# kit4b/kit4b

Measured on AMD Instinct MI355X. Metric: Mreads/sec aligned (100 bp SE vs 3 Gbp .sfx), higher is better.
Workload: dtype u64

## Files before the change

### kit4b_amd/csrc/k4_align.hip

```cpp
#include <stdlib.h>
#include <type_traits>
#include "k4_align_common.h"

#define K4_BS(nch) ((nch) >= 16 ? 128 : 256)
template <int NCH>
struct K4Lane {
  const uint64_t* rd;
  uint32_t* ded;
  const uint32_t* sup;
  const uint64_t* ent;
  uint64_t* memo;
  static constexpr int NW = NCH + 1;
  K4_DEV uint64_t word(int s, int c) const { return rd[(s * NW + c) * K4_BS(NCH)]; }
  K4_DEV uint64_t chunk_at(int s, int o) const {
    int w = o >> 5, sh = 2 * (o & 31);
    uint64_t hi = word(s, w);
    if (!sh) return hi;
    return (hi << sh) | (word(s, w + 1) >> (64 - sh));
  }
};

struct K4Probe {
  int cmp;
  int mm;
// ... 110 lines not shown
      more = cnt == PFN;
      bool memo_hit = false, memo_pending = false;
      int memo_mm = 0;
#pragma unroll
      for (int j = 0; j < PFN; j++) {
        if (j < cnt) {
          if (!CAPTURE && j == 0 && first_group && tshift == 0 && (sizeof(KT) == 4 || cl >= kk + 2)) {
            const uint64_t mv = ln.memo[s * K4_BS(NCH)];
            const int kind = (int)(mv >> 62), fm = (int)((mv >> 48) & 0x3FFF), mmv = (int)((mv >> 40) & 0xFF);
            if (kind == 1 || (kind == 2 && fm < cl)) continue;
            if (kind == 2 && mmv != 0xFF) {
              lb0[0] = 0; lb1[0] = 1; ps0[0] = (RT)(mv & 0xFFFFFFFFFFull);
              memo_hit = true; memo_mm = mmv;
              continue;
            }
          }
          const uint64_t code = ln.chunk_at(s, oo[j]) >> (64 - 2 * kk);
          uint64_t sub;
          {
            KT e_lb0, e_ps0, e_lb1;
            k4d_ktab_fetch<KT>(ix, code << tshift, (code + 1) << tshift, e_lb0, e_ps0, sig[j], e_lb1, sub,
                               sizeof(KT) == 8 && tshift == 0 && cl >= kk + 2);
            lb0[j] = (RT)e_lb0; ps0[j] = (RT)e_ps0; lb1[j] = (RT)e_lb1;
          }
          if (CAPTURE && defer_deep && tshift == 0 && (uint64_t)(lb1[j] - lb0[j]) > K4_DEFER_BUCKET) return K4_DEFER;
          if (a.deep_general && (!CAPTURE || a.deep_general == 1) && tshift == 0 && (uint64_t)(lb1[j] - lb0[j]) > K4_DEFER_BUCKET) return K4_NEED_SLOW;
          if (sizeof(KT) == 8 && tshift == 0 && cl >= kk + 2 && sub != K4_KTAB64_IRREGULAR) {
            uint32_t before, count;
            k4d_ktab_sub(sub, (uint32_t)(ln.chunk_at(s, oo[j] + kk) >> 60), before, count);
            if (before) ps0[j] = (RT)NOPOS;
            lb0[j] += (RT)before;
            lb1[j] = lb0[j] + (RT)count;
          }
          if (CAPTURE && j == 0 && first_group && tshift == 0) {
            if (lb1[0] == lb0[0]) ln.memo[s * K4_BS(NCH)] = k4d_memo_pack(1, 0, 0, 0);
            else memo_pending = lb1[0] == lb0[0] + 1;
          }
          if (sizeof(KT) == 4 && tshift == 0 && lb1[j] == lb0[j] + 1 && cl > kk) {
            const int nb = min(K4_SIG_BASES32, cl - kk);
            const uint32_t cb = (uint32_t)(ln.chunk_at(s, oo[j] + kk) >> 32);
            const uint32_t df = (cb ^ sig[j]) & (0xFFFFFFFFu << (32 - 2 * nb));
            if (df) {
              lb1[j] = lb0[j];
              if (CAPTURE && j == 0 && first_group) {
                ln.memo[s * K4_BS(NCH)] = k4d_memo_pack(2, (uint64_t)ps0[0], 0xFF, kk + (__clz(df) >> 1));
                memo_pending = false;
              }
            }
          }
        }
      }
      uint32_t touch = 0;
#pragma unroll
      for (int j = 0; j < PFN; j++)
        if (j < cnt && tshift == 0 && lb1[j] > lb0[j] && !(j == 0 && memo_hit) && (sizeof(KT) == 4 || (uint64_t)ps0[j] != NOPOS))
          touch |= ix.ref2[((int64_t)ps0[j] - oo[j]) >> 4];

#pragma unroll
      for (int j = 0; j < PFN; j++) {
        if (j >= cnt || stop) continue;
        const int o = oo[j];
        n_lookup++;
        int64_t lo = (int64_t)lb0[j];
        int64_t hi = (int64_t)lb1[j] - 1;
        const int64_t bucket_hi = hi;
        int64_t found = -1;
        uint64_t fpos = 0;
        int fmm = 0;
        while (lo <= hi) {
          const int64_t mid = (lo + hi) >> 1;
          const uint64_t p = (tshift == 0 && mid == (int64_t)lb0[j] && (sizeof(KT) == 4 || (uint64_t)ps0[j] != NOPOS))
                                 ? (uint64_t)ps0[j] : k4d_sa_at<EL>(ix, (uint64_t)mid);
          K4Probe pr;
          if (!CAPTURE && j == 0 && memo_hit) { pr.cmp = 0; pr.mm = memo_mm; pr.fm = len; pr.exc = false; }
          else {
            pr = k4d_probe<NCH>(ix, ln, s, o, cl, len, p);
            n_probe++;
            if (CAPTURE && j == 0 && memo_pending) ln.memo[s * K4_BS(NCH)] = k4d_memo_pack(2, p, pr.mm > 254 ? 254 : pr.mm, pr.fm);
          }
          if (pr.exc) return K4_NEED_SLOW;
          if (pr.cmp > 0) lo = mid + 1;
          else {
            if (pr.cmp == 0) { found = mid; fpos = p; fmm = pr.mm; }
            hi = mid - 1;
          }
        }
        if (found != lo) continue;
        int64_t idx = found;
        uint64_t p = fpos;
        int mm = fmm;
        int iter = 0;
        bool first = true;
        while (!max_iter || iter < max_iter) {
          if (!first) {
            if (idx >= bucket_hi || idx + 1 >= n) break;
            const uint64_t p2 = k4d_sa_at<EL>(ix, (uint64_t)idx + 1);
            if ((int64_t)p2 + cl > n) break;
            const K4Probe pr = k4d_probe<NCH>(ix, ln, s, o, cl, len, p2);
            n_probe++;
            if (pr.exc) return K4_NEED_SLOW;
            if (pr.cmp != 0) break;
            idx += 1; p = p2; mm = pr.mm;
          }
          first = false;
          if (p < (uint64_t)o) continue;
          const uint64_t left = p - (uint64_t)o;
          int e;
          uint64_t e_start, e_end;
          if (ix.n_entries <= K4_LDS_ENTRIES) {
            int lo_e = 0, hi_e = (int)ix.n_entries - 1;
            e = -1; e_start = 0; e_end = 0;
            while (hi_e >= lo_e) {
              const int mid_e = (hi_e + lo_e) >> 1;
              const uint64_t sv = ln.ent[mid_e];
              if (sv > left) { hi_e = mid_e - 1; continue; }
              const uint64_t ev = ln.ent[K4_LDS_ENTRIES + mid_e];
              if (ev >= left) { e = mid_e; e_start = sv; e_end = ev; break; }
              lo_e = mid_e + 1;
            }
          } else {
            e = k4d_map_entry(ix, left);
            e_start = e >= 0 ? ix.ent_start[e] : 0;
            e_end = e >= 0 ? ix.ent_end[e] : 0;
          }
          if (e < 0 || left + (uint64_t)len - 1 > e_end) continue;
          const uint32_t targ_id = (uint32_t)(1 + p - (uint32_t)o);
          bool dup = false;
          for (int q = 0; q < n_ded; q++) dup |= (ln.ded[q * K4_BS(NCH)] == targ_id);
          if (dup) continue;
          if (n_ded >= K4_DEDUP_CAP) return K4_NEED_SLOW;
          ln.ded[n_ded * K4_BS(NCH)] = targ_id;
          n_ded++;
          iter++;
          n_cand++;
          if (mm > allow_mm || mm >= st.nxt) continue;
          k4d_fold(st, mm, hits, rp.max_hits, ix.ent_id[e], (uint32_t)(left - e_start), len, strand_c);
          if (st.inst > rp.max_hits && st.low == 0) break;
        }
        if (st.inst > rp.max_hits && st.low == 0) stop = true;
      }
      if (touch == 0x5A5A5A5Au && len < 0) n_probe++;
      first_group = false;
    }
  }
  return k4d_lcm_result(*p_inst, *p_low, p_nxt, st, rp.mm_delta, rp.max_hits, p_inst, p_low);
}

K4_DEV uint64_t k4d_rev2(uint64_t x) {
  uint64_t y = __brevll(x);
  return ((y & 0x5555555555555555ull) << 1) | ((y >> 1) & 0x5555555555555555ull);
}

template <int NCH>
K4_DEV uint32_t k4d_pack_read(const uint8_t* __restrict__ src, int len, uint64_t* col, uint32_t& n_ns) {
  constexpr int NW = NCH + 1;
  uint32_t fl = 0;
  n_ns = 0;
  const uint32_t sh = (uint32_t)(reinterpret_cast<uintptr_t>(src) & 3);
  const uint32_t* __restrict__ src32 = reinterpret_cast<const uint32_t*>(src - sh);
  const int span = len + (int)sh;
#pragma unroll
  for (int c = 0; c < NCH; c++) {
    uint64_t acc = 0;
    if (32 * c < len) {
      uint32_t dq[9] = {0, 0, 0, 0, 0, 0, 0, 0, 0};
      if (c * 32 + 32 <= span) {
        uint32_t d8[8];
        k4d_load_words<8>(src32 + c * 8, d8);
#pragma unroll
        for (int q = 0; q < 8; q++) dq[q] = d8[q];
      } else {
#pragma unroll
        for (int q = 0; q < 8; q++)
          if (c * 32 + q * 4 < span) dq[q] = src32[c * 8 + q];
      }
      if (c * 32 + 32 < span) dq[8] = src32[c * 8 + 8];
#pragma unroll
      for (int q = 0; q < 8; q++) {
        const int base = c * 32 + q * 4;
        uint32_t d = __builtin_amdgcn_alignbyte(dq[q + 1], dq[q], sh);
        d &= 0x07070707u;
        if (base + 4 > len) d &= len > base ? (0xFFFFFFFFu >> (8 * (4 - (len - base)))) : 0u;
        const uint32_t hi4 = d & 0x04040404u;
        if (hi4) {
          const uint32_t inval = hi4 & ((d << 1) | (d << 2)) & 0x04040404u;
          if (inval) fl |= K4_RF_INVALID;
          n_ns += __popc(hi4 & ~inval);
          d &= ~(hi4 | (hi4 >> 1) | (hi4 >> 2));
        }
        acc = (acc << 8) | ((d & 3) << 6) | (((d >> 8) & 3) << 4) | (((d >> 16) & 3) << 2) | ((d >> 24) & 3);
      }
    }
    col[c * K4_BS(NCH)] = acc;
  }
  col[NCH * K4_BS(NCH)] = 0;
  if (n_ns) fl |= K4_RF_HAS_N;
#pragma unroll
  for (int c = 0; c < NCH; c++) {
    uint64_t r = 0;
    if (32 * c < len) {
      const int o = len - 32 * (c + 1);
      uint64_t f;
      if (o >= 0) {
        const int w = o >> 5, sh = 2 * (o & 31);
        const uint64_t hi = col[w * K4_BS(NCH)];
        f = sh ? (hi << sh) | (col[(w + 1) * K4_BS(NCH)] >> (64 - sh)) : hi;
      } else
        f = col[0] >> (2 * (-o));
      r = k4d_rev2(~f) & k4d_range_mask(0, len - 32 * c);
    }
    col[(NW + c) * K4_BS(NCH)] = r;
  }
  col[(NW + NCH) * K4_BS(NCH)] = 0;
  return fl;
}

template <int EL, int NCH, bool FIRST, typename KT, bool DEFER = false>
__global__ void __launch_bounds__(K4_BS(NCH), (NCH >= 16 ? K4_STEP_WAVES_LONG : NCH >= 8 ? K4_STEP_WAVES_MID : NCH == 5 ? K4_STEP_WAVES_5 : K4_STEP_WAVES)) k4k_align_step(K4AlignArgs a, int step, const uint32_t* __restrict__ in_ids,
                                                      const uint64_t* __restrict__ in_rows,
                                                      const uint32_t* __restrict__ in_count, uint32_t* __restrict__ out_ids,
                                                      uint64_t* __restrict__ out_rows, uint32_t* __restrict__ out_count) {
  extern __shared__ uint64_t lds[];
  constexpr int NW = NCH + 1;
  const int tid = threadIdx.x;
  const int lane = tid & 63;
  K4Lane<NCH> ln;
  ln.rd = lds + tid;
  ln.ded = reinterpret_cast<uint32_t*>(lds + 2 * NW * K4_BS(NCH)) + tid;
  ln.memo = lds + 2 * NW * K4_BS(NCH) + (K4_DEDUP_CAP * K4_BS(NCH)) / 2 + tid;
  uint64_t* ent_l = lds + 2 * NW * K4_BS(NCH) + (K4_DEDUP_CAP * K4_BS(NCH)) / 2 + 2 * K4_BS(NCH);
  uint32_t* sup_l = reinterpret_cast<uint32_t*>(ent_l + 2 * K4_LDS_ENTRIES);
  ln.ent = ent_l;
  ln.sup = sup_l;
  for (int q = tid; q < K4_SUP_WORDS; q += K4_BS(NCH)) sup_l[q] = a.ix.excsup[q];
  if (a.ix.n_entries <= K4_LDS_ENTRIES)
    for (int q = tid; q < (int)a.ix.n_entries; q += K4_BS(NCH)) {
      ent_l[q] = a.ix.ent_start[q];
      ent_l[K4_LDS_ENTRIES + q] = a.ix.ent_end[q];
    }
  __syncthreads();
  uint64_t* col = lds + tid;
  uint32_t n_lookup = 0, n_probe = 0, n_cand = 0, n_slow = 0, n_bases = 0, n_done = 0;
  const int64_t count = (FIRST && !(DEFER && in_ids != nullptr)) ? a.n_reads : (int64_t)*in_count;
  const int64_t stride = (int64_t)gridDim.x * K4_BS(NCH);
  uint32_t ch_cur = 0, ch_left = 0;
  const bool from_list = !FIRST || (DEFER && in_ids != nullptr);
  const bool may_defer = DEFER && FIRST && in_ids == nullptr && a.defer_ids != nullptr;
  uint32_t dch_cur = 0, dch_left = 0;
  for (int64_t jb = (int64_t)blockIdx.x * K4_BS(NCH) + (tid & ~63); jb < count; jb += stride) {
    const int64_t j = jb + lane;
    bool active = j < count;
    int64_t i = 0;
    if (active) {
      i = from_list ? (int64_t)in_ids[j] : j;
      if (from_list && (uint32_t)i == K4_NO_READ) active = false;
    }
    bool slow = false, survive = false, deferred = false;
    int ext_from = -1;
    if (active) {
      const int len = (int)a.lens[i];
      const K4ReadParams rp = k4d_read_params(a, len);
      bool skip = false;
      if (FIRST) {
        if (!from_list) {
          n_done++;
          n_bases += (uint32_t)len;
        }
        uint32_t fl = 0, n_ns = 0;
        if (len < 1 || len > 32 * NCH || len > K4_MAX_FAST_READ_LEN) {
          fl = K4_RF_TOOLONG;
          if (a.mode == 1) {
            const uint8_t* src = a.reads + a.offs[i];
            for (int q = 0; q < len; q++) {
              uint32_t b = src[q] & 7;
              if (b == 4) n_ns++; else if (b > 4) fl |= K4_RF_INVALID;
            }
          }
        } else
          fl = k4d_pack_read<NCH>(a.reads + a.offs[i], len, col, n_ns);
        if (a.mode == 1) {
          int max_ns = 0;
          if (a.kp.max_ns) max_ns = max((len * a.kp.max_ns) / 100, a.kp.max_ns);
          if ((fl & K4_RF_INVALID) || (int)n_ns > max_ns) {
            k4_read_result r = {K4_HR_SEQERRS, 0, 0, 0, K4_NAR_NS, 0};
            a.rr[i] = r;
            if (!a.sparse_hits)
              for (int q = 0; q < a.max_hits; q++) *reinterpret_cast<uint4*>(&a.hits[i * a.max_hits + q]) = make_uint4(0, 0, 0, 0);
            skip = true;
          }
        }
        slow = fl != 0 && !skip;
        if (((a.mode == 1 && a.kp.pe_mode == 4) || a.best) && !skip) slow = true;
      } else {
        const uint64_t* row = in_rows + (int64_t)j * K4_ROW_WORDS(NCH);
        {
          const k4_u64x2_a8 mv = *reinterpret_cast<const k4_u64x2_a8*>(row + 2 * NCH);
          ln.memo[0] = mv.x; ln.memo[K4_BS(NCH)] = mv.y;
        }
        uint64_t rw[2 * NCH];
#pragma unroll
        for (int c = 0; c < NCH; c++) {
          const k4_u64x2_a8 v = *reinterpret_cast<const k4_u64x2_a8*>(row + 2 * c);
          rw[2 * c] = v.x; rw[2 * c + 1] = v.y;
        }
#pragma unroll
        for (int c = 0; c < NCH; c++) {
          col[c * K4_BS(NCH)] = rw[c];
          col[(NW + c) * K4_BS(NCH)] = rw[NCH + c];
        }
        col[NCH * K4_BS(NCH)] = 0;
        col[(NW + NCH) * K4_BS(NCH)] = 0;
      }
      if (!skip && (rp.core_len < 1 || rp.max_hits < 1 || rp.max_hits > a.max_hits)) slow = true;
      if (!skip && !slow) {
        int n_esc = 0;
        if (rp.tot_mm > 0)
          for (; n_esc <= rp.tot_mm; n_esc++)
            if (len / (n_esc + rp.mm_delta) <= rp.core_len) break;
        const bool has_final = rp.tot_mm > 0 ? n_esc <= rp.tot_mm : true;
        const int n_phases = n_esc + (has_final ? 1 : 0);
        int allow, cl, delta;
        if (step < n_esc) { allow = step; cl = len / (step + rp.mm_delta); delta = cl; }
        else { allow = rp.tot_mm; cl = rp.core_len; delta = rp.core_delta; }
        k4_hit* hits = a.hits + i * a.max_hits;
        int inst = 0, low = 0, nxt = 0;
        const uint32_t c0 = n_lookup, c1 = n_probe, c2 = n_cand;
        if (FIRST) { ln.memo[0] = K4_MEMO_NONE; ln.memo[K4_BS(NCH)] = K4_MEMO_NONE; }
        int rslt = k4d_lcm_fast<EL, NCH, KT, FIRST>(a, ln, len, allow, cl, delta, rp, &inst, &low, &nxt, hits, n_lookup, n_probe, n_cand, DEFER && may_defer);
        if (rslt == K4_NEED_SLOW) {
          slow = true;
          n_lookup = c0; n_probe = c1; n_cand = c2;
        }
        else if (DEFER && rslt == K4_DEFER) {
          deferred = true;
          n_lookup = c0; n_probe = c1; n_cand = c2;
        }
        else if (rslt == 0 && step + 1 >= n_phases && a.ext_on) { slow = true; ext_from = n_phases; }
        else if (rslt != 0 || step + 1 >= n_phases) k4d_finalize(a, i, len, rp, rslt, inst, low, nxt);
        else survive = true;
      }
      if (slow) {
        k4d_push_slow(a, i, ext_from >= 0 ? ext_from : step);
        n_slow++;
      }
    }
    if (FIRST && DEFER) {
      const unsigned long long dm = __ballot(deferred);
      const uint32_t dcnt = (uint32_t)__popcll(dm);
      if (dcnt) {
        if (dcnt > dch_left) {
          for (uint32_t q = lane; q < dch_left; q += 64) a.defer_ids[dch_cur + q] = K4_NO_READ;
          uint32_t base = 0;
          if (lane == 0) base = atomicAdd(&a.ctl[K4_CTL_DEFER], (uint32_t)K4_CHUNK);
          dch_cur = __shfl(base, 0, 64);
          dch_left = K4_CHUNK;
        }
        if (deferred) a.defer_ids[dch_cur + (uint32_t)__popcll(dm & ((1ull << lane) - 1ull))] = (uint32_t)i;
        dch_cur += dcnt;
        dch_left -= dcnt;
      }
    }
    const unsigned long long m = __ballot(survive);
    const uint32_t cnt = (uint32_t)__popcll(m);
    if (cnt) {
      if (cnt > ch_left) {
        for (uint32_t q = lane; q < ch_left; q += 64) out_ids[ch_cur + q] = K4_NO_READ;
        uint32_t base = 0;
        if (lane == 0) base = atomicAdd(out_count, (uint32_t)K4_CHUNK);
        ch_cur = __shfl(base, 0, 64);
        ch_left = K4_CHUNK;
      }
      if (survive) {
        const uint32_t slot = ch_cur + (uint32_t)__popcll(m & ((1ull << lane) - 1ull));
        out_ids[slot] = (uint32_t)i;
        uint64_t* row = out_rows + (int64_t)slot * K4_ROW_WORDS(NCH);
#pragma unroll
        for (int c = 0; c < NCH; c++) {
          k4_u64x2_a8 v;
          const int w0 = 2 * c, w1 = 2 * c + 1;
          v.x = w0 < NCH ? col[w0 * K4_BS(NCH)] : col[(NW + w0 - NCH) * K4_BS(NCH)];
          v.y = w1 < NCH ? col[w1 * K4_BS(NCH)] : col[(NW + w1 - NCH) * K4_BS(NCH)];
          *reinterpret_cast<k4_u64x2_a8*>(row + 2 * c) = v;
        }
        {
          k4_u64x2_a8 mv;
          mv.x = ln.memo[0]; mv.y = ln.memo[K4_BS(NCH)];
          *reinterpret_cast<k4_u64x2_a8*>(row + 2 * NCH) = mv;
        }
      }
      ch_cur += cnt;
      ch_left -= cnt;
    }
  }
  for (uint32_t q = lane; q < ch_left; q += 64) out_ids[ch_cur + q] = K4_NO_READ;
  if (FIRST && DEFER)
    for (uint32_t q = lane; q < dch_left; q += 64) a.defer_ids[dch_cur + q] = K4_NO_READ;
  {
    unsigned long long v[6] = {n_done, n_lookup, n_probe, n_cand, n_slow, n_bases};
#pragma unroll
    for (int q = 0; q < 6; q++) {
      unsigned long long x = v[q];
      for (int d = 32; d > 0; d >>= 1) x += __shfl_down(x, d, 64);
      if (lane == 0 && x) atomicAdd(&a.counters[q], x);
    }
  }
}

static uint32_t next_pow2(uint64_t v) {
  uint32_t p = 1;
  while (p < v) p <<= 1;
  return p;
}

static size_t k4_survivor_slots(size_t cap) {
  static_assert(K4_CHUNK * 7 >= 8 * 63, "cap / 7 must cover the abandoned chunk tails");
  return cap + cap / 7 + (size_t)2048 * 4 * K4_CHUNK + K4_CHUNK;
}

static int nch_for(int max_len) {
  if (max_len <= 128) return 4;
  if (max_len <= 160) return 5;
  if (max_len <= 256) return 8;
  return 16;
}

extern "C" int k4_reserve(k4_index* ix, int64_t max_reads, int32_t max_read_len, int32_t max_hits) {
  if (!ix || max_reads < 0 || max_read_len < 1 || max_hits < 1) return K4_ERR_PARAMS;
  if (max_read_len > K4_MAX_READ_LEN) return k4_fail(ix, K4_ERR_PARAMS, "read length %d exceeds %d", max_read_len, K4_MAX_READ_LEN);
  if (max_reads >= 0xFFFFFFF0ll) return k4_fail(ix, K4_ERR_PARAMS, "at most 2^32-16 reads per batch");
  K4_HIP(ix, hipSetDevice(ix->device));
  K4Workspace& w = ix->ws;
  bool touched = false;
  int fast_len = std::min<int>(max_read_len, K4_MAX_FAST_READ_LEN);
  if (max_reads > w.cap_reads || fast_len > w.cap_len) {
    int64_t cap = std::max<int64_t>(max_reads, w.cap_reads);
    cap = (cap + 255) / 256 * 256;
    int len = std::max(fast_len, w.cap_len);
    int nch = nch_for(len);
    touched = true;
    w.cap_reads = 0;
    w.cap_len = 0;
    for (void* q : {(void*)w.ids[0], (void*)w.ids[1], (void*)w.rows[0], (void*)w.rows[1], (void*)w.slow_list, (void*)w.slow_step,
                    (void*)w.huge_list, (void*)w.huge_step})
      if (q) hipFree(q);
    w.ids[0] = w.ids[1] = nullptr; w.rows[0] = w.rows[1] = nullptr; w.slow_list = nullptr; w.slow_step = nullptr;
    w.huge_list = nullptr; w.huge_step = nullptr;
    const size_t slots = k4_survivor_slots((size_t)cap);
    for (int b = 0; b < 2; b++) {
      K4_HIP(ix, hipMalloc(&w.ids[b], slots * 4));
      K4_HIP(ix, hipMalloc(&w.rows[b], slots * K4_ROW_WORDS(nch) * 8));
    }
    K4_HIP(ix, hipMalloc(&w.slow_list, (size_t)cap * 4));
    K4_HIP(ix, hipMalloc(&w.slow_step, (size_t)cap));
    K4_HIP(ix, hipMalloc(&w.huge_list, (size_t)cap * 4));
    K4_HIP(ix, hipMalloc(&w.huge_step, (size_t)cap));
    w.cap_reads = cap;
    w.cap_len = len;
  }
  if (!w.ctl) {
    touched = true;
    K4_HIP(ix, hipMalloc(&w.ctl, K4_CTL_WORDS * 4));
    K4_HIP(ix, hipMemset(w.ctl, 0, K4_CTL_WORDS * 4));
  }
  uint64_t nodes = ix->d.max_iter ? std::min<uint64_t>((uint64_t)ix->d.max_iter * 48, K4_MAX_IDENT_NODES) : K4_MAX_IDENT_NODES;
  uint32_t hcap = next_pow2(std::max<uint64_t>(2 * nodes + 2, 1024));
  if (!w.slow_hash || hcap > w.slow_hash_cap) {
    touched = true;
    if (w.slow_hash) hipFree(w.slow_hash);
    w.slow_hash = nullptr;
    const size_t words = (size_t)K4_SLOW_WAVES * K4_SMALL_HASH + (size_t)K4_HUGE_WAVES * hcap;
    const size_t bytes = words * 8 + (size_t)(K4_SLOW_WAVES + K4_HUGE_WAVES) * 4;
    K4_HIP(ix, hipMalloc(&w.slow_hash, bytes));
    K4_HIP(ix, hipMemset(w.slow_hash, 0, bytes));
    w.slow_hash_cap = hcap;
    w.slow_lanes = K4_SLOW_WAVES;
  }
  w.cap_hits = std::max(w.cap_hits, max_hits);
  if (touched) K4_HIP(ix, hipDeviceSynchronize());
  return K4_OK;
}

template <int EL, int NCH, typename KT>
static int launch_steps(k4_index* ix, K4AlignArgs& a, int n_steps, hipStream_t st) {
  K4Workspace& w = ix->ws;
  const size_t lds = (size_t)2 * (NCH + 1) * K4_BS(NCH) * 8 + (size_t)K4_DEDUP_CAP * K4_BS(NCH) * 4 + (size_t)2 * K4_BS(NCH) * 8 + (size_t)2 * K4_LDS_ENTRIES * 8 +
                     (size_t)K4_SUP_WORDS * 4 + 16;
  if (lds > 48 * 1024) {
    K4_HIP(ix, hipFuncSetAttribute((const void*)k4k_align_step<EL, NCH, true, KT, false>, hipFuncAttributeMaxDynamicSharedMemorySize, (int)lds));
    K4_HIP(ix, hipFuncSetAttribute((const void*)k4k_align_step<EL, NCH, true, KT, true>, hipFuncAttributeMaxDynamicSharedMemorySize, (int)lds));
    K4_HIP(ix, hipFuncSetAttribute((const void*)k4k_align_step<EL, NCH, false, KT>, hipFuncAttributeMaxDynamicSharedMemorySize, (int)lds));
  }
  const unsigned full = 256 * 8 * (256 / K4_BS(NCH));
  const bool timed = ix->timing && ix->ev_used < 4096;
  if (timed) {
    if (ix->ev_used == ix->ev0.size()) {
      hipEvent_t e0, e1, e2;
      K4_HIP(ix, hipEventCreate(&e0));
      K4_HIP(ix, hipEventCreate(&e1));
      K4_HIP(ix, hipEventCreate(&e2));
      ix->ev0.push_back(e0);
      ix->ev1.push_back(e1);
      ix->ev2.push_back(e2);
    }
    K4_HIP(ix, hipEventRecord(ix->ev0[ix->ev_used], st));
  }
  unsigned grid0 = (unsigned)std::min<int64_t>((a.n_reads + K4_BS(NCH) - 1) / K4_BS(NCH), full);
  static const int deep_mode = getenv("K4_DEEP_TO_GENERAL") ? atoi(getenv("K4_DEEP_TO_GENERAL")) : 0;
  a.deep_general = (deep_mode && ix->deep_bucket_frac >= K4_DEFER_MIN_FRAC) ? deep_mode : 0;
  if (ix->deep_bucket_frac >= K4_DEFER_MIN_FRAC && a.deep_general != 1) {
    a.defer_ids = w.ids[1];
    hipLaunchKernelGGL((k4k_align_step<EL, NCH, true, KT, true>), dim3(grid0), dim3(K4_BS(NCH)), lds, st, a, 0, (const uint32_t*)nullptr,
                       (const uint64_t*)nullptr, (const uint32_t*)nullptr, w.ids[0], w.rows[0], w.ctl + 2);
    hipLaunchKernelGGL((k4k_align_step<EL, NCH, true, KT, true>), dim3(grid0), dim3(K4_BS(NCH)), lds, st, a, 0, (const uint32_t*)w.ids[1],
                       (const uint64_t*)nullptr, (const uint32_t*)(w.ctl + K4_CTL_DEFER), w.ids[0], w.rows[0], w.ctl + 2);
  } else {
    a.defer_ids = nullptr;
    hipLaunchKernelGGL((k4k_align_step<EL, NCH, true, KT, false>), dim3(grid0), dim3(K4_BS(NCH)), lds, st, a, 0, (const uint32_t*)nullptr,
                       (const uint64_t*)nullptr, (const uint32_t*)nullptr, w.ids[0], w.rows[0], w.ctl + 2);
  }
  for (int t = 1; t < n_steps; t++) {
    const int in = (t - 1) & 1, out = t & 1;
    hipLaunchKernelGGL((k4k_align_step<EL, NCH, false, KT>), dim3(grid0), dim3(K4_BS(NCH)), lds, st, a, t, w.ids[in], w.rows[in],
                       w.ctl + 2 + (t - 1), w.ids[out], w.rows[out], w.ctl + 2 + t);
  }
  if (timed) K4_HIP(ix, hipEventRecord(ix->ev1[ix->ev_used], st));
  return K4_OK;
}

template <int EL, typename KT>
static int launch_all(k4_index* ix, K4AlignArgs& a, int max_len, int n_steps, hipStream_t st) {
  K4Workspace& w = ix->ws;
  const int nch = nch_for(std::min(max_len, K4_MAX_FAST_READ_LEN));
  if (nch > nch_for(w.cap_len)) return k4_fail(ix, K4_ERR_INTERNAL, "workspace not reserved for read length %d", max_len);
  if (n_steps < 1 || n_steps > K4_CTL_WORDS - 4) return k4_fail(ix, K4_ERR_INTERNAL, "bad phase count %d", n_steps);
  a.slow_list = w.slow_list;
  a.slow_step = w.slow_step;
  a.ctl = w.ctl;
  a.counters = (unsigned long long*)ix->counters;
  a.huge_list = w.huge_list;
  a.huge_step = w.huge_step;
  a.slow_probe = nullptr;
  a.slow_hash = w.slow_hash;
  a.slow_hash_cap = w.slow_hash_cap;
  a.slow_gen = reinterpret_cast<uint32_t*>(w.slow_hash + (size_t)K4_SLOW_WAVES * K4_SMALL_HASH + (size_t)K4_HUGE_WAVES * w.slow_hash_cap);
  a.nw = nch + 1;
  if (a.n_reads == 0) return K4_OK;
  K4_HIP(ix, hipMemsetAsync(w.ctl, 0, K4_CTL_WORDS * 4, st));
  int rc;
  switch (nch) {
    case 4: rc = launch_steps<EL, 4, KT>(ix, a, n_steps, st); break;
    case 5: rc = launch_steps<EL, 5, KT>(ix, a, n_steps, st); break;
    case 8: rc = launch_steps<EL, 8, KT>(ix, a, n_steps, st); break;
    default: rc = launch_steps<EL, 16, KT>(ix, a, n_steps, st); break;
  }
  if (rc != K4_OK) return rc;
  rc = k4i_launch_general(ix, a, max_len, st);
  if (rc != K4_OK) return rc;
  if (ix->timing && ix->ev_used < ix->ev0.size() && ix->ev_used < 4096) {
    K4_HIP(ix, hipEventRecord(ix->ev2[ix->ev_used], st));
    ix->ev_used++;
  }
  K4_HIP(ix, hipGetLastError());
  return K4_OK;
}

static int run_dev(k4_index* ix, K4AlignArgs& a, int max_len, void* stream) {
  K4Workspace& w = ix->ws;
  if (a.n_reads > w.cap_reads || std::min(max_len, K4_MAX_FAST_READ_LEN) > w.cap_len || a.max_hits > w.cap_hits ||
      !w.slow_hash || !w.ids[0] || !w.ids[1] || !w.rows[0] || !w.rows[1] || !w.slow_list || !w.huge_list || !w.ctl)
    return k4_fail(ix, K4_ERR_PARAMS, "k4_reserve(%lld, %d, %d) must precede the *_dev call", (long long)a.n_reads,
                   max_len, a.max_hits);
  a.ix = ix->d;
  hipStream_t st = (hipStream_t)stream;
  {
    const int mc = a.mode == 0 ? a.ap.min_chimeric_len : a.kp.min_chimeric_len;
    const int mi = a.mode == 0 ? a.ap.micro_indel_len : a.kp.micro_indel_len;
    const int ms = a.mode == 0 ? a.ap.max_splice_junct_len : a.kp.max_splice_junct_len;
    if (mc < 0 || mi < 0 || mi > 20 || ms < 0 || (ms != 0 && (ms < 25 || ms > 100000)))
      return k4_fail(ix, K4_ERR_PARAMS, "MinChimericLen / microInDelLen (0..20) / MaxSpliceJunctLen (0, 25..100000) out of range");
    a.ext_on = (mc > 0 || mi > 0 || ms > 0) ? 1 : 0;
    if ((mi > 0 || ms > 0) && !a.seg2)
      return k4_fail(ix, K4_ERR_PARAMS, "microInDel / splice phases report two segments: use the *_ext entry points (k4_seg2 output)");
    if (a.ext_on && (a.best || (a.mode == 1 && a.kp.pe_mode == 4)))
      return k4_fail(ix, K4_ERR_PARAMS, "the optional AlignReads phases cannot be combined with LocateBestMatches (-N)");
    if (a.seg2 && a.n_reads > 0) K4_HIP(ix, hipMemsetAsync(a.seg2, 0, (size_t)a.n_reads * sizeof(k4_seg2), st));
  }
  int tot_mm = a.ap.tot_mm;
  if (a.mode == 1) {
    tot_mm = a.kp.max_subs == 0 ? 0 : std::max(1, (int)(0.5 + (max_len * a.kp.max_subs) / 100.0));
    tot_mm = std::min(tot_mm, 63);
  }
  const int n_steps = tot_mm + 1;
  if (ix->d.el == 4) return ix->d.ktab64 ? launch_all<4, uint64_t>(ix, a, max_len, n_steps, st) : launch_all<4, uint32_t>(ix, a, max_len, n_steps, st);
  return ix->d.ktab64 ? launch_all<5, uint64_t>(ix, a, max_len, n_steps, st) : launch_all<5, uint32_t>(ix, a, max_len, n_steps, st);
}

static int check_align_params(k4_index* ix, const k4_align_params* p) {
  if (!p) return K4_ERR_PARAMS;
  if (p->tot_mm < 0 || p->tot_mm > 63 || p->core_len < 1 || p->core_delta < 0 || p->max_core_slides < 1 ||
      p->mm_delta < 1 || p->strand < 0 || p->strand > 2 || p->max_hits < 1 || p->max_hits > 4096)
    return k4_fail(ix, K4_ERR_PARAMS, "AlignReads parameters out of range");
  return K4_OK;
}

extern "C" int k4_align_reads_batch_dev(k4_index* ix, const k4_align_params* p, int64_t n, int32_t max_len,
                                        const void* d_reads, const void* d_offs, const void* d_lens, void* d_rslt,
                                        void* d_inst, void* d_low, void* d_nxt, void* d_hits, void* stream) {
  return k4_align_reads_ext_batch_dev(ix, p, n, max_len, d_reads, d_offs, d_lens, d_rslt, d_inst, d_low, d_nxt, d_hits, nullptr, stream);
}
extern "C" int k4_align_reads_ext_batch_dev(k4_index* ix, const k4_align_params* p, int64_t n, int32_t max_len,
                                            const void* d_reads, const void* d_offs, const void* d_lens, void* d_rslt,
                                            void* d_inst, void* d_low, void* d_nxt, void* d_hits, void* d_seg2, void* stream) {
  if (!ix) return K4_ERR_PARAMS;
  int rc = check_align_params(ix, p);
  if (rc != K4_OK) return rc;
  if (n < 0 || (n > 0 && (!d_reads || !d_offs || !d_lens || !d_rslt || !d_inst || !d_low || !d_nxt || !d_hits)))
    return k4_fail(ix, K4_ERR_PARAMS, "null buffer");
  K4AlignArgs a;
  memset(&a, 0, sizeof(a));
  a.reads = (const uint8_t*)d_reads; a.offs = (const uint64_t*)d_offs; a.lens = (const uint32_t*)d_lens;
  a.n_reads = n; a.mode = 0; a.ap = *p;
  a.rslt = (int32_t*)d_rslt; a.inst = (int32_t*)d_inst; a.low = (int32_t*)d_low; a.nxt = (int32_t*)d_nxt;
  a.hits = (k4_hit*)d_hits; a.max_hits = p->max_hits;
  a.seg2 = (k4_seg2*)d_seg2;
  return run_dev(ix, a, max_len, stream);
}

extern "C" int k4_best_matches_batch_dev(k4_index* ix, const k4_align_params* p, int64_t n, int32_t max_len, const void* d_reads,
                                         const void* d_offs, const void* d_lens, void* d_rslt, void* d_inst, void* d_hits,
                                         void* stream) {
  if (!ix) return K4_ERR_PARAMS;
  int rc = check_align_params(ix, p);
  if (rc != K4_OK) return rc;
  if (n < 0 || (n > 0 && (!d_reads || !d_offs || !d_lens || !d_rslt || !d_inst || !d_hits))) return k4_fail(ix, K4_ERR_PARAMS, "null buffer");
  K4AlignArgs a;
  memset(&a, 0, sizeof(a));
  a.reads = (const uint8_t*)d_reads; a.offs = (const uint64_t*)d_offs; a.lens = (const uint32_t*)d_lens;
  a.n_reads = n; a.mode = 0; a.best = 1; a.ap = *p;
  a.rslt = (int32_t*)d_rslt; a.inst = (int32_t*)d_inst;
  a.hits = (k4_hit*)d_hits; a.max_hits = p->max_hits;
  return run_dev(ix, a, max_len, stream);
}

static int resolve_kalign(k4_index* ix, const k4_kalign_params* p, k4_kalign_params* out) {
  if (!p) return K4_ERR_PARAMS;
  *out = *p;
  if (p->max_subs < 0 || p->max_subs > 15 || (p->min_edit_dist != 1 && p->min_edit_dist != 2) || p->max_ns < 0 ||
      p->strand < 0 || p->strand > 2 || p->max_ml < 1 || p->max_ml > 4096 || p->pe_mode < 0 || p->pe_mode > 4)
    return k4_fail(ix, K4_ERR_PARAMS, "kalign parameters out of range");
  int slides = 0;
  int mcl = k4_min_core_len(ix, p->pmode, &slides);
  if (out->min_core_len <= 0) out->min_core_len = mcl;
  if (out->max_num_slides <= 0) out->max_num_slides = slides;
  return K4_OK;
}

int k4i_kalign_batch_dev(k4_index* ix, const k4_kalign_params* p, int64_t n, int32_t max_len, const void* d_reads,
                         const void* d_offs, const void* d_lens, void* d_out, void* d_hits, void* stream, int sparse_hits);
extern "C" int k4_kalign_batch_dev(k4_index* ix, const k4_kalign_params* p, int64_t n, int32_t max_len,
                                   const void* d_reads, const void* d_offs, const void* d_lens, void* d_out,
                                   void* d_hits, void* stream) {
// ... 281 lines not shown
```

### kit4b_amd/csrc/k4_align_common.h

```cpp
#pragma once
#include <stdio.h>
#include <string.h>
#include <algorithm>
#include "k4_device.h"

#define K4_NEED_SLOW (-100)
#define K4_DEFER (-101)
#define K4_RF_HAS_N 1u
#define K4_RF_INVALID 2u
#define K4_RF_TOOLONG 4u
#ifndef K4_STEP_WAVES
#define K4_STEP_WAVES 4
#endif
#ifndef K4_STEP_WAVES_LONG
#define K4_STEP_WAVES_LONG 2
#endif
#ifndef K4_STEP_WAVES_5
#define K4_STEP_WAVES_5 4
#endif
#ifndef K4_STEP_WAVES_MID
#define K4_STEP_WAVES_MID 3
#endif
#define K4_CHUNK 512
#define K4_NO_READ 0xFFFFFFFFu
#define K4_ROW_WORDS(nch) (2 * (nch) + 2)
#ifndef K4_PF
#define K4_PF 4
#endif
#ifndef K4_PF5
#define K4_PF5 4
#endif
#ifndef K4_SLOW_WAVES_PER_EU
#define K4_SLOW_WAVES_PER_EU 4
#endif
#ifndef K4_SLOW_WAVES_PER_EU_EXT
#define K4_SLOW_WAVES_PER_EU_EXT 3
#endif
#ifndef K4_DEFER_BUCKET
#define K4_DEFER_BUCKET K4_DEEP_BUCKET
#endif
#define K4_DEFER_MIN_FRAC 0.002
#ifndef K4_SLOW_KB
#define K4_SLOW_KB 1
#endif
#ifndef K4_SLOW_WAVES
#define K4_SLOW_WAVES 8192
#endif
#define K4_SMALL_HASH 4096
#define K4_HUGE_WAVES 256
#define K4_CTL_HUGE 68
#define K4_CTL_DEFER 70
#define K4_CTL_WORDS 72

struct K4AlignArgs {
  K4DevIndex ix;
  const uint8_t* reads;
  const uint64_t* offs;
  const uint32_t* lens;
  int64_t n_reads;
  int32_t mode;
  int32_t sparse_hits;
  int32_t best;
  int32_t deep_general;
  k4_align_params ap;
  k4_kalign_params kp;
  int32_t* rslt;
  int32_t* inst;
  int32_t* low;
  int32_t* nxt;
  k4_read_result* rr;
  k4_hit* hits;
  k4_seg2* seg2;
  int32_t ext_on;
  int32_t max_hits;
  uint32_t* slow_list;
  uint8_t* slow_step;
  uint32_t* huge_list;
  uint8_t* huge_step;
  uint32_t* defer_ids;
  uint32_t* ctl;
  unsigned long long* counters;
  uint8_t* slow_probe;
  uint64_t* slow_hash;
  uint32_t* slow_gen;
  uint32_t slow_hash_cap;
  int32_t nw;
};

struct K4ReadParams {
  int tot_mm, core_len, core_delta, max_slides, mm_delta, strand, max_hits;
  int min_core_len, min_chimeric_len, micro_indel_len, max_splice_junct_len;
};

struct K4State {
  int inst, low, nxt, cur_hit;
};

K4_DEV K4ReadParams k4d_read_params(const K4AlignArgs& a, int len) {
  K4ReadParams p;
  if (a.mode == 0) {
    p.tot_mm = a.ap.tot_mm; p.core_len = a.ap.core_len; p.core_delta = a.ap.core_delta;
    p.max_slides = a.ap.max_core_slides; p.mm_delta = a.ap.mm_delta; p.strand = a.ap.strand;
    p.max_hits = a.ap.max_hits;
    p.min_core_len = a.ap.min_core_len; p.min_chimeric_len = a.ap.min_chimeric_len;
    p.micro_indel_len = a.ap.micro_indel_len; p.max_splice_junct_len = a.ap.max_splice_junct_len;
    return p;
  }
  int mm = a.kp.max_subs == 0 ? 0 : (int)(0.5 + (len * a.kp.max_subs) / 100.0);
  if (a.kp.max_subs != 0 && mm < 1) mm = 1;
  if (mm > 63) mm = 63;
  int cl = len / (a.kp.min_edit_dist == 1 ? mm + 1 : mm + 2);
  if (cl < a.kp.min_core_len) cl = a.kp.min_core_len;
  int sl = (a.kp.max_num_slides * len + 99) / 100;
  if (sl < 1) sl = 1;
  int cd = len / sl - 1;
  if (cd < cl) cd = cl;
  p.tot_mm = mm; p.core_len = cl; p.core_delta = cd; p.max_slides = sl;
  p.mm_delta = a.kp.min_edit_dist; p.strand = a.kp.strand; p.max_hits = a.kp.max_ml < 1 ? 1 : a.kp.max_ml;
  p.min_core_len = a.kp.min_core_len; p.min_chimeric_len = a.kp.min_chimeric_len;
  p.micro_indel_len = a.kp.micro_indel_len; p.max_splice_junct_len = a.kp.max_splice_junct_len;
  return p;
}

K4_DEV void k4d_store_hit(k4_hit* h, uint32_t chrom_id, uint32_t loci, int len, char strand, int mm, uint32_t ext = 0) {
  uint4 v;
  v.x = chrom_id;
  v.y = loci;
  v.z = (uint32_t)(len & 0xFFFF) | ((uint32_t)(uint8_t)strand << 16) | ((uint32_t)(mm & 0xFF) << 24);
  v.w = ext;
  *reinterpret_cast<uint4*>(h) = v;
}

K4_DEV void k4d_fold(K4State& st, int mm, k4_hit* hits, int max_hits, uint32_t chrom_id, uint32_t loci, int len,
                     char strand) {
  if (mm < st.low) {
    st.cur_hit = 0;
    st.inst = 1;
    st.nxt = st.low;
    st.low = mm;
    if (hits) k4d_store_hit(&hits[0], chrom_id, loci, len, strand, mm);
  } else if (mm == st.low) {
    st.inst += 1;
    if (st.cur_hit != -1 && st.inst <= max_hits) {
      st.cur_hit += 1;
      if (hits && st.cur_hit < max_hits) k4d_store_hit(&hits[st.cur_hit], chrom_id, loci, len, strand, mm);
    }
  } else if (mm < st.nxt)
    st.nxt = mm;
}

K4_DEV int k4d_lcm_result(int p_inst, int p_low, int* p_nxt, const K4State& st, int mm_delta, int max_hits,
                          int* o_inst, int* o_low) {
  if (p_low == st.low && p_inst == st.inst) {
    if (*p_nxt > st.nxt) {
      *p_nxt = st.nxt;
      if (st.nxt - p_low < mm_delta) return K4_HR_MMDELTA;
      return K4_HR_RMMDELTA;
    }
    return K4_HR_NONE;
  }
  *o_low = st.low; *o_inst = st.inst; *p_nxt = st.nxt;
  if (st.inst >= 1 && (st.nxt - st.low) < mm_delta) return K4_HR_MMDELTA;
  if (st.inst > max_hits) return K4_HR_HITINSTS;
  return K4_HR_HITS;
}

K4_DEV void k4d_finalize(const K4AlignArgs& a, int64_t i, int len, const K4ReadParams& rp, int rslt, int inst,
                         int low, int nxt) {
  k4_hit* hits = a.hits + i * a.max_hits;
  int nvalid = (rslt == K4_HR_HITS || rslt == K4_HR_MMDELTA || rslt == K4_HR_HITINSTS) ? min(inst, rp.max_hits) : 0;
  if (!a.sparse_hits)
    for (int q = nvalid; q < a.max_hits; q++) *reinterpret_cast<uint4*>(&hits[q]) = make_uint4(0, 0, 0, 0);
  if (a.mode == 0) {
    a.rslt[i] = rslt; a.inst[i] = inst;
    if (a.low) a.low[i] = low;
    if (a.nxt) a.nxt[i] = nxt;
    return;
  }
  k4_read_result r;
  if (inst > rp.max_hits) inst = rp.max_hits + 1;
  if (a.kp.pe_mode >= 3 && rslt == K4_HR_HITINSTS) { inst = rp.max_hits; rslt = K4_HR_HITS; }
  r.hit_rslt = rslt; r.inst = inst; r.low_mm = low; r.nxt_mm = nxt; r.nar = K4_NAR_NOHIT; r.num_hits = 0;
  switch (rslt) {
    case K4_HR_NONE: r.inst = 0; r.low_mm = 0; r.nxt_mm = 0; break;
    case K4_HR_HITS:
      if (a.kp.pe_mode >= 2) { r.nar = K4_NAR_ACCEPTED; r.num_hits = min(inst, rp.max_hits); }
      else if (!a.kp.pe_mode || inst == 1) { r.nar = K4_NAR_ACCEPTED; r.num_hits = 1; }
      else { r.nar = K4_NAR_MULTIALIGN; r.num_hits = inst; }
      break;
    case K4_HR_MMDELTA: r.nar = K4_NAR_MMDELTA; break;
    case K4_HR_HITINSTS: r.nar = K4_NAR_MULTIALIGN; break;
    default: break;
  }
  (void)len;
  a.rr[i] = r;
}

K4_DEV void k4d_push_slow(const K4AlignArgs& a, int64_t i, int step) {
  uint32_t slot = atomicAdd(&a.ctl[0], 1u);
  a.slow_list[slot] = (uint32_t)i;
  a.slow_step[slot] = (uint8_t)step;
}

int k4i_launch_general(k4_index* ix, K4AlignArgs& a, int max_len, hipStream_t st);
```

Measured before the change: 3072.

## Stage contiguous read bytes cooperatively per wave through LDS before packing

For short-read kernels (NCH 4 or 5) on the first step, each wavefront loads the contiguous byte span covering its 64 reads with coalesced 16-byte loads. It packs the bases into 2-bit words in the dedup/memo LDS region and records per-piece masks for N or invalid bases. Lanes whose read is clean then assemble their forward chunks from LDS, and only the reverse complement is computed per lane. This replaces scattered, misaligned per-lane global loads, at the cost of extra ballots, wave barriers, reuse of LDS, and a fallback path when reads are not contiguous or contain Ns. It is enabled by default through an environment variable.

```diff
diff --git a/kit4b_amd/csrc/k4_align.hip b/kit4b_amd/csrc/k4_align.hip
--- a/kit4b_amd/csrc/k4_align.hip
+++ b/kit4b_amd/csrc/k4_align.hip
@@ -286,8 +286,7 @@
 }
 
 template <int NCH>
-K4_DEV uint32_t k4d_pack_read(const uint8_t* __restrict__ src, int len, uint64_t* col, uint32_t& n_ns) {
-  constexpr int NW = NCH + 1;
+K4_DEV uint32_t k4d_pack_fwd(const uint8_t* __restrict__ src, int len, uint64_t* col, uint32_t& n_ns) {
   uint32_t fl = 0;
   n_ns = 0;
   const uint32_t sh = (uint32_t)(reinterpret_cast<uintptr_t>(src) & 3);
@@ -327,8 +326,14 @@
     }
     col[c * K4_BS(NCH)] = acc;
   }
+  if (n_ns) fl |= K4_RF_HAS_N;
+  return fl;
+}
+
+template <int NCH>
+K4_DEV void k4d_pack_rc(int len, uint64_t* col) {
+  constexpr int NW = NCH + 1;
   col[NCH * K4_BS(NCH)] = 0;
-  if (n_ns) fl |= K4_RF_HAS_N;
 #pragma unroll
   for (int c = 0; c < NCH; c++) {
     uint64_t r = 0;
@@ -346,7 +351,108 @@
     col[(NW + c) * K4_BS(NCH)] = r;
   }
   col[(NW + NCH) * K4_BS(NCH)] = 0;
+}
+
+template <int NCH>
+K4_DEV uint32_t k4d_pack_read(const uint8_t* __restrict__ src, int len, uint64_t* col, uint32_t& n_ns) {
+  const uint32_t fl = k4d_pack_fwd<NCH>(src, len, col, n_ns);
+  k4d_pack_rc<NCH>(len, col);
   return fl;
+}
+
+#define K4_STAGE_WORDS (K4_DEDUP_CAP * 64 + 2 * 128)
+#define K4_STAGE_MASKS 12
+#ifndef K4_STAGE_BATCH
+#define K4_STAGE_BATCH 4
+#endif
+#define K4_STAGE_PIECES (K4_STAGE_WORDS - 2 * K4_STAGE_MASKS)
+static_assert(K4_STAGE_PIECES >= (64 * 150 + 15 + 15) / 16, "64 reads of 150 bp at any alignment must fit");
+static_assert((K4_STAGE_PIECES + 63) / 64 + 1 <= K4_STAGE_MASKS && K4_STAGE_PIECES % 2 == 0, "mask words");
+
+template <int NCH>
+K4_DEV int k4d_stage_at(int w, int wave) {
+  const int g = w >> 6, h = g - K4_DEDUP_CAP;
+  const int row = h < 0 ? g * K4_BS(NCH) + wave * 64 : (K4_DEDUP_CAP + 2 * (h >> 1)) * K4_BS(NCH) + wave * 128 + (h & 1) * 64;
+  return row + (w & 63);
+}
+
+K4_DEV uint32_t k4d_pack4(uint32_t d) { return (d & 0x03030303u) * 0x40100401u; }
+
+template <int NCH>
+K4_DEV bool k4d_stage_wave(const uint8_t* __restrict__ reads, bool active, uint64_t off, int len, uint32_t* sb, int wave, int lane,
+                           uint64_t* col) {
+  constexpr int ROUNDS = (2 * NCH + 1) < (K4_STAGE_PIECES + 63) / 64 ? (2 * NCH + 1) : (K4_STAGE_PIECES + 63) / 64;
+  const unsigned long long am = __ballot(active);
+  if (!am) return false;
+  const int n_act = __popcll(am);
+  if (am != (~0ull >> (64 - n_act))) return false;
+  const uint64_t p = (uint64_t)reinterpret_cast<uintptr_t>(reads) + off;
+  const uint64_t base = (((uint64_t)__builtin_amdgcn_readfirstlane((uint32_t)(p >> 32)) << 32) | __builtin_amdgcn_readfirstlane((uint32_t)p)) & ~15ull;
+  const uint64_t rel64 = p - base;
+  const bool fits = active && len >= 1 && len <= 32 * NCH && rel64 < 16ull * K4_STAGE_PIECES && rel64 + (uint64_t)len <= 16ull * K4_STAGE_PIECES;
+  const uint32_t rel = fits ? (uint32_t)rel64 : 0u, end = fits ? (uint32_t)rel64 + (uint32_t)len : 0u;
+  const uint32_t prel = __shfl_up(rel, 1, 64), pend = __shfl_up(end, 1, 64);
+  const bool ok = !active || (fits && (lane == 0 || (rel > prel && end >= pend && rel <= pend + 15u)));
+  if (__ballot(ok) != ~0ull) return false;
+  const int n_pieces = (int)((__builtin_amdgcn_readlane(end, n_act - 1) + 15u) >> 4);
+  const uint4* __restrict__ src = reinterpret_cast<const uint4*>(static_cast<uintptr_t>(base));
+  uint64_t my_mask = 0;
+#pragma unroll
+  for (int r0 = 0; r0 < ROUNDS; r0 += K4_STAGE_BATCH) {
+    uint4 v[K4_STAGE_BATCH];
+#pragma unroll
+    for (int q = 0; q < K4_STAGE_BATCH; q++) {
+      const int r = r0 + q;
+      v[q] = make_uint4(0, 0, 0, 0);
+      if (r < ROUNDS && r * 64 < n_pieces && r * 64 + lane < n_pieces) v[q] = src[r * 64 + lane];
+    }
+#pragma unroll
+    for (int q = 0; q < K4_STAGE_BATCH; q++) {
+      const int r = r0 + q;
+      if (r < ROUNDS && r * 64 < n_pieces) {
+        const bool have = r * 64 + lane < n_pieces;
+        const uint32_t word = (k4d_pack4(v[q].x) & 0xFF000000u) | ((k4d_pack4(v[q].y) >> 8) & 0x00FF0000u) |
+                              ((k4d_pack4(v[q].z) >> 16) & 0x0000FF00u) | (k4d_pack4(v[q].w) >> 24);
+        if (have) sb[k4d_stage_at<NCH>(r * 64 + lane, wave)] = word;
+        const unsigned long long bm = __ballot(have && ((v[q].x | v[q].y | v[q].z | v[q].w) & 0x04040404u) != 0u);
+        if (lane == r) my_mask = bm;
+      }
+    }
+  }
+  uint64_t* mk = reinterpret_cast<uint64_t*>(sb + k4d_stage_at<NCH>(K4_STAGE_PIECES, wave));
+  if (lane < K4_STAGE_MASKS) mk[lane] = my_mask;
+  __builtin_amdgcn_fence(__ATOMIC_RELEASE, "wavefront");
+  __builtin_amdgcn_wave_barrier();
+  __builtin_amdgcn_fence(__ATOMIC_ACQUIRE, "wavefront");
+  bool staged = false;
+  if (active) {
+    const int w0 = (int)(rel >> 4), shb = (int)(rel & 15u), span = (int)((end - 1u) >> 4) - w0;
+    const int mi = w0 >> 6, ms = w0 & 63;
+    const uint64_t m0 = mk[mi], m1 = mk[mi + 1];
+    const uint64_t mv = ms ? (m0 >> ms) | (m1 << (64 - ms)) : m0;
+    if (!(mv & ((2ull << span) - 1ull))) {
+      const int a0 = k4d_stage_at<NCH>(w0, wave), a1 = k4d_stage_at<NCH>((w0 | 63) + 1, wave) + (w0 & 63) - 64;
+      uint32_t wv[2 * NCH + 1];
+#pragma unroll
+      for (int k = 0; k < 2 * NCH + 1; k++) wv[k] = 16 * k < shb + len ? sb[((w0 & 63) + k < 64 ? a0 : a1) + k] : 0u;
+      const uint32_t sh = 2u * (uint32_t)shb;
+#pragma unroll
+      for (int c = 0; c < NCH; c++) {
+        uint64_t f = 0;
+        if (32 * c < len) {
+          const uint64_t hi = ((uint64_t)wv[2 * c] << 32) | wv[2 * c + 1];
+          f = sh ? (hi << sh) | (wv[2 * c + 2] >> (32 - sh)) : hi;
+          f &= k4d_range_mask(0, len - 32 * c);
+        }
+        col[c * K4_BS(NCH)] = f;
+      }
+      staged = true;
+    }
+  }
+  __builtin_amdgcn_fence(__ATOMIC_RELEASE, "wavefront");
+  __builtin_amdgcn_wave_barrier();
+  __builtin_amdgcn_fence(__ATOMIC_ACQUIRE, "wavefront");
+  return staged;
 }
 
 template <int EL, int NCH, bool FIRST, typename KT, bool DEFER = false>
@@ -391,6 +497,12 @@
     }
     bool slow = false, survive = false, deferred = false;
     int ext_from = -1;
+    bool staged = false;
+    if (FIRST && (NCH == 4 || NCH == 5)) {
+      if (!from_list && a.stage_reads)
+        staged = k4d_stage_wave<NCH>(a.reads, active, active ? a.offs[i] : 0ull, active ? (int)a.lens[i] : 0,
+                                     reinterpret_cast<uint32_t*>(lds + 2 * NW * K4_BS(NCH)), tid >> 6, lane, col);
+    }
     if (active) {
       const int len = (int)a.lens[i];
       const K4ReadParams rp = k4d_read_params(a, len);
@@ -410,7 +522,9 @@
               if (b == 4) n_ns++; else if (b > 4) fl |= K4_RF_INVALID;
             }
           }
-        } else
+        } else if (staged)
+          k4d_pack_rc<NCH>(len, col);
+        else
           fl = k4d_pack_read<NCH>(a.reads + a.offs[i], len, col, n_ns);
         if (a.mode == 1) {
           int max_ns = 0;
@@ -641,6 +755,8 @@
   unsigned grid0 = (unsigned)std::min<int64_t>((a.n_reads + K4_BS(NCH) - 1) / K4_BS(NCH), full);
   static const int deep_mode = getenv("K4_DEEP_TO_GENERAL") ? atoi(getenv("K4_DEEP_TO_GENERAL")) : 0;
   a.deep_general = (deep_mode && ix->deep_bucket_frac >= K4_DEFER_MIN_FRAC) ? deep_mode : 0;
+  static const int stage_reads = getenv("K4_STAGE_READS") ? atoi(getenv("K4_STAGE_READS")) : 1;
+  a.stage_reads = stage_reads;
   if (ix->deep_bucket_frac >= K4_DEFER_MIN_FRAC && a.deep_general != 1) {
     a.defer_ids = w.ids[1];
     hipLaunchKernelGGL((k4k_align_step<EL, NCH, true, KT, true>), dim3(grid0), dim3(K4_BS(NCH)), lds, st, a, 0, (const uint32_t*)nullptr,
diff --git a/kit4b_amd/csrc/k4_align_common.h b/kit4b_amd/csrc/k4_align_common.h
--- a/kit4b_amd/csrc/k4_align_common.h
+++ b/kit4b_amd/csrc/k4_align_common.h
@@ -62,6 +62,7 @@
   int32_t sparse_hits;
   int32_t best;
   int32_t deep_general;
+  int32_t stage_reads;
   k4_align_params ap;
   k4_kalign_params kp;
   int32_t* rslt;
```

Result: slower. 3040 (-1.0%).
